# yweweler/single-speaker-tts

Hardware: AMD Instinct MI355X
Metric: mel-frames/sec (end-to-end text->waveform incl. 60-iter Griffin-Lim, 64-utt LJ-Speech-shaped batch per GPU) (higher is better)
Workload: dtype f32

## Files before the change

### include/sstts_hip.h

```cpp
#ifndef SSTTS_HIP_H
#define SSTTS_HIP_H

#include <stddef.h>
#include <stdint.h>

#ifdef __cplusplus
extern "C" {
#endif

typedef struct tts_handle_s* tts_handle_t;

enum tts_status {
    TTS_OK = 0,
    TTS_ERR_INVALID = -1,
    TTS_ERR_NOT_LOADED = -2,
    TTS_ERR_HIP = -3,
    TTS_ERR_DB_RANGE = -4,
    TTS_ERR_UNSUPPORTED = -5
};

typedef struct tts_config {
    int32_t struct_size;
    int32_t vocabulary_size;
    int32_t embedding_size;
// ... 129 lines not shown

int tts_synthesize_host(tts_handle_t h, const int32_t* ids_host, int B, int Ts, const tts_synth_params_t* p,
                        int* ticket);
int tts_wait_host(tts_handle_t h, int ticket, const float** wav_host, size_t* n_floats);
int tts_wait_host_outputs(tts_handle_t h, int ticket, const float** linear_host, size_t* n_linear, const float** align_host,
                          size_t* n_align);

int tts_profile_reset(tts_handle_t h);
int tts_decoder_kernel_choice(tts_handle_t h, int B, int T_sent, int pipelined);
int tts_debug_workspace(tts_handle_t h, const char* name, void** dptr, size_t* bytes);
int tts_debug_gl_plan(int T, int B, int win_length, int hop_length, int n_workers, int* items, int max_items, int* ring_frames);
int tts_debug_gl_plan_ragged(const int32_t* n_frames, int B, int win_length, int hop_length, int n_workers,
                             int* items, int max_items, int* ring_frames);
int tts_debug_gemm(tts_handle_t h, const float* A, const float* Wt, float* C, int M, int N, int Cin, int ktaps, int T,
                   int pool);
int tts_debug_hold(tts_handle_t h, int n_wgs, int lds_kb, double ms);
int tts_profile_get(tts_handle_t h, const char* stage, float* ms_total, int64_t* launches);
int tts_device_info(tts_handle_t h, char uuid_hex[33], int* n_compute_units);

#ifdef __cplusplus
}
#endif
#endif
```

### single-speaker-tts_amd/_hip.py

```python
import ctypes
import os
from ctypes import (POINTER, byref, c_char_p, c_float, c_int, c_int32, c_int64, c_size_t, c_uint64,
                    c_void_p)

import numpy as np

_HERE = os.path.dirname(os.path.abspath(__file__))
LIB_PATH = os.environ.get('SSTTS_HIP_LIB') or os.path.join(_HERE, 'libsstts_hip.so')

TTS_OK = 0
TTS_ERR_INVALID = -1
TTS_ERR_NOT_LOADED = -2
TTS_ERR_HIP = -3
TTS_ERR_DB_RANGE = -4
TTS_ERR_UNSUPPORTED = -5


class TtsError(RuntimeError):
    def __init__(self, code, msg):
        super().__init__('sstts_hip error {}: {}'.format(code, msg))
        self.code = code


class TtsConfig(ctypes.Structure):
# ... 74 lines not shown
    'tts_default_feature_params': (c_int, [POINTER(TtsFeatureParams)]),
    'tts_plan_features': (c_int, [c_void_p, c_void_p, c_void_p, c_int, POINTER(TtsFeatureParams), c_void_p]),
    'tts_extract_features': (c_int, [c_void_p, c_void_p, c_void_p, c_int, POINTER(TtsFeatureParams), c_void_p, c_void_p,
                                     c_void_p]),
    'tts_synthesize': (c_int, [c_void_p, c_void_p, c_int, c_int, POINTER(TtsSynthParams), c_void_p, c_void_p,
                               c_void_p, c_void_p, c_void_p]),
    'tts_synthesize_host': (c_int, [c_void_p, c_void_p, c_int, c_int, POINTER(TtsSynthParams), POINTER(c_int)]),
    'tts_wait_host': (c_int, [c_void_p, c_int, POINTER(c_void_p), POINTER(c_size_t)]),
    'tts_wait_host_outputs': (c_int, [c_void_p, c_int, POINTER(c_void_p), POINTER(c_size_t), POINTER(c_void_p), POINTER(c_size_t)]),
    'tts_profile_reset': (c_int, [c_void_p]),
    'tts_profile_get': (c_int, [c_void_p, c_char_p, POINTER(c_float), POINTER(c_int64)]),
    'tts_decoder_kernel_choice': (c_int, [c_void_p, c_int, c_int, c_int]),
    'tts_debug_workspace': (c_int, [c_void_p, c_char_p, POINTER(c_void_p), POINTER(c_size_t)]),
    'tts_debug_hold': (c_int, [c_void_p, c_int, c_int, ctypes.c_double]),
    'tts_debug_gemm': (c_int, [c_void_p, c_void_p, c_void_p, c_void_p, c_int, c_int, c_int, c_int, c_int, c_int]),
    'tts_debug_gl_plan': (c_int, [c_int, c_int, c_int, c_int, c_int, POINTER(c_int), c_int, POINTER(c_int)]),
    'tts_debug_gl_plan_ragged': (c_int, [POINTER(c_int32), c_int, c_int, c_int, c_int, POINTER(c_int), c_int, POINTER(c_int)]),
    'tts_device_info': (c_int, [c_void_p, c_char_p, POINTER(c_int)]),
}

_lib = None


def exported_symbols():
    return sorted(_PROTOTYPES)


def load_library(path=None):
    global _lib
    if _lib is not None and path is None:
# ... 551 lines not shown
```

### single-speaker-tts_amd/csrc/api_handle.hip

```cpp
#include "api_internal.h"

namespace tts_api {
thread_local std::string g_create_error;
const char* const kStageNames[ST_COUNT] = {"encoder", "decoder", "postnet", "denorm", "gl_iter", "gl_final", "debug_gemm", "eval_loss", "features"};
}

namespace tts_api {


int fail(tts_handle_t h, int code, const std::string& msg) {
    if (h) h->err = msg;
    else g_create_error = msg;
    return code;
}


const char* kAtt = "decoder2/decoder/output_projection_wrapper/multi_rnn_cell/cell_0/attention_wrapper";

const char* kMrc = "decoder2/decoder/output_projection_wrapper/multi_rnn_cell";


std::string bn_name(int i) {
    return i == 0 ? std::string("batch_normalization") : "batch_normalization_" + std::to_string(i);
}
// ... 635 lines not shown
int tts_set_option(tts_handle_t h, const char* key, int value) {
    DeviceScope dev_scope(h);
    if (!h || !key) return TTS_ERR_INVALID;
    if (!std::strcmp(key, "use_graph")) {
        int have = 0;
        if (value && !(value == 2 && h->debug_hooks) && !graph_runtime_ok(&have))
            return fail(h, TTS_ERR_UNSUPPORTED,
                        "use_graph: this process runs the library on HIP runtime " + std::to_string(have) + ", older than the " +
                        std::to_string(HIP_VERSION) + " it was built with (a libamdhip64 loaded before the library, e.g. the one "
                        "PyTorch bundles); hipGraph replays of the decoder are wrong there (csrc/api_internal.h, `use_graph`) -- the "
                        "launches are enqueued directly instead");
        h->use_graph = value;
    }
    else if (!std::strcmp(key, "profile")) h->profile = value;
    else if (!std::strcmp(key, "fused_tail")) h->fused_tail = value;
    else if (!std::strcmp(key, "persistent_decoder")) {
        if (value != h->persistent_decoder) {
            int rc = sync_all(h);
            if (rc) return rc;
        }
        h->persistent_decoder = value;
    }
    else if (!std::strcmp(key, "gl_pair")) h->gl_pair = value;
    else if (!std::strcmp(key, "gl_momentum")) {
        if (value < 0 || value > 999) return fail(h, TTS_ERR_INVALID, "gl_momentum: thousandths of the momentum, 0 .. 999");
        h->gl_momentum = value;
    }
    else if (!std::strcmp(key, "gl_wide_from")) h->gl_wide = value < -2 ? -2 : value;
    else if (!std::strcmp(key, "pd_ws")) {
        if (value != h->pd_ws) {
// ... 350 lines not shown
```

### single-speaker-tts_amd/csrc/api_internal.h

```cpp
#pragma once
#include <cmath>
#include <cstdio>
#include <cstring>
#include <memory>
#include <mutex>
#include <optional>
#include <string>
#include <utility>
#include <vector>
#include "decoder.h"
#include "griffin_lim.h"
#include "tts_common.h"
#include <algorithm>
#include <map>

namespace tts_api {
using namespace tts;


constexpr int TTS_MAX_N_MELS = 1024;
constexpr int TTS_MAX_FIELD = 1 << 20;
constexpr long long TTS_MAX_WEIGHT_FLOATS = (1ll << 30) - 5;

extern thread_local std::string g_create_error;
// ... 156 lines not shown
    }
};

}
using namespace tts_api;

struct tts_handle_s {
    tts_config_t cfg;
    int device = 0;
    hipStream_t stream = nullptr;
    bool own_stream = false;
    std::string err;
    int use_graph = 0;
    int fused_tail = 1;
    bool tail_configured = false;
    int profile = 0;
    int pipeline = 1;
    int reserve_cus = 32;
    int hold_lds_kb = 64;
    int enc_stream = 1;
    CallPipeline pl;
    int persistent_decoder = 1;
    int pd_ws = 1;
    bool ws_configured = false;
    int gl_pair = 3;
    int gl_momentum = 0;
    int gl_wide = -1;
    int n_cus_dev = 0;
    bool pd_configured = false;
    int debug_hooks = 0;
// ... 199 lines not shown
```

### single-speaker-tts_amd/csrc/api_pipeline.hip

```cpp
#include "api_internal.h"

namespace tts_api {


int gl_wide_from(tts_handle_t h, int B, int Ts, int n_steps, int T, int n_iter) {
    if (h->gl_wide == -2 || h->reserve_cus <= 0) return -1;
    const int pd = pd_choice(h, B, Ts, h->reserve_cus, true);
    if (pd == 0) return -1;
    if (h->gl_wide >= 0) return h->gl_wide;
    if (pd != 2) return -1;
    const int per_launch = h->gl_momentum > 0 ? 1 : (h->gl_pair < 1 ? 1 : (h->gl_pair > 3 ? 3 : h->gl_pair));
    if (h->n_cus_dev != 256 || h->n_cus_dev - h->reserve_cus < 16) return -1;
    const double launch_ms = 3.125e-6 * (double)B * T * per_launch * 224.0 / (double)(h->n_cus_dev - h->reserve_cus);
    const double step_ms = (0.0356 + 0.0089 * (double)Ts / 150.0) * (h->cfg.force_cudnn ? 0.038 / 0.045 : 1.0);
    const double dec_ms = step_ms * n_steps + 0.1;
    const int n_launches = (n_iter + per_launch - 1) / per_launch;
    const int from = (int)std::ceil((dec_ms + 0.5 * launch_ms + 0.1) / launch_ms);
    return from <= n_launches ? from : -1;
}

struct SynthCall {
    const int32_t* ids;
    int B, Ts;
    const tts_synth_params_t* sp;
// ... 171 lines not shown
    args.project_later = k.pipelined;
    args.parity = parity;
    args.keys = k.pipelined ? k.keys_ahead : nullptr;
    if ((rc = decoder_impl(h, k.memory, B, Ts, k.sp->n_steps, k.mel, k.align_out, nullptr, args, &k.proj))) return rc;
    if (k.pipelined) HIPCHK(h, pl.dec_done[parity].record(pl.front));
    else if (pl.front) HIPCHK(h, pl.serial_done.record(on.main_stream));
    return TTS_OK;
}

static int synth_main(tts_handle_t h, SynthCall& k) {
    auto& pl = h->pl;
    const tts_synth_params_t* sp = k.sp;
    const int B = k.B, T = k.T, parity = k.parity;
    int rc = TTS_OK;
    const bool phase_on_front = k.gl_streaming && k.pipelined && sp->n_iter >= 0 && (k.init_phase != nullptr || sp->n_iter == 0);
    if (k.pipelined) {
        if (k.hold_flag) HIPCHK(h, hipMemsetAsync(k.hold_flag, 1, sizeof(int), pl.front));
        if (phase_on_front) {
            HIPCHK(h, pl.gl_done[parity].wait(pl.front));
            HIPCHK(h, launch_phase_init(pl.front, k.init_phase, sp->seed, k.phase_pair[0], B, k.F, T, k.FP));
        }
        HIPCHK(h, pl.front_done.record(pl.front));
        HIPCHK(h, pl.front_done.wait(h->stream));
    }
    if (k.proj && (rc = run_single(h, *k.proj))) return rc;
    if (pl.encs) HIPCHK(h, pl.gap[parity].record(h->stream));
    int* db_flag = nullptr;
    if (denorm_can_assert(sp->ref_db, sp->max_db) && (rc = denorm_flag_arm(h, &db_flag))) return rc;
    if ((rc = postnet_impl(h, k.mel, B, T, k.linear_out, k.magi, sp->ref_db, sp->max_db, sp->power, db_flag))) return rc;
    if (db_flag && (rc = denorm_flag_read(h))) return rc;
    if (pl.front) HIPCHK(h, pl.post_done[parity].record(h->stream));
    const int wide_from = (k.pipelined && k.gl_streaming) ? gl_wide_from(h, B, k.Ts, sp->n_steps, T, sp->n_iter) : -1;
    pl.gl_wide_used[parity] = wide_from >= 0;
    if (k.gl_streaming)
        rc = gl_run(h, k.magi, k.init_phase, sp->seed, B, T, sp->n_iter, sp->win_length, sp->hop_length, h->cfg.n_fft, k.wav, nullptr,
                    sp->peak_normalize != 0, k.pipelined, k.phase_pair, phase_on_front, wide_from);
    else
        rc = gl_run_generic(h, k.magi, k.init_phase, sp->seed, B, T, sp->n_iter, sp->win_length, sp->hop_length, h->cfg.n_fft, k.wav,
                            nullptr, sp->peak_normalize != 0);
    if (pl.front && !rc) HIPCHK(h, pl.gl_done[parity].record(h->stream));
    return rc;
}

static int synthesize_impl(tts_handle_t h, const int32_t* ids, int B, int Ts, const tts_synth_params_t* sp, const float* init_phase,
                           float* wav, float* mel_out, float* align_out, float* linear_out, const StageArgs& host) {
    int rc = check_ready(h);
    if (rc) return rc;
// ... 146 lines not shown
```

### single-speaker-tts_amd/csrc/api_stages.hip

```cpp
#include "api_internal.h"

namespace tts_api {


int run_cbhg(tts_handle_t h, const CbhgWeights& w, const char* tag, const float* x, int B, int T, float* out,
             int64_t* launches) {
    const tts_config_t& c = h->cfg;
    const int M = B * T;
    const int NB = w.n_banks, NF = w.n_filters;
    const int U = c.n_highway_units, H = c.n_gru_units;
    const std::string t(tag);
    WS(h, (t + ".bank").c_str(), float, (size_t)M * NB * NF, bank);
    WS(h, (t + ".p1").c_str(), float, (size_t)M * w.proj_filters[0], p1);
    WS(h, (t + ".p2").c_str(), float, (size_t)M * w.proj_filters[1], p2);
    WS(h, (t + ".hw0").c_str(), float, (size_t)M * U, hw0);
    WS(h, (t + ".hw1").c_str(), float, (size_t)M * U, hw1);
    WS(h, (t + ".xproj").c_str(), float, (size_t)M * 6 * H, xproj);

    for (int k0 = 0; k0 < NB; k0 += TTS_GEMM_MAX_GROUPS) {
        GemmBatch b;
        std::memset(&b, 0, sizeof(b));
        const int ng = std::min(TTS_GEMM_MAX_GROUPS, NB - k0);
        for (int i = 0; i < ng; ++i) {
            const int k = k0 + ng - 1 - i;
            b.g[i] = conv_group(x, w.c_in, k + 1, T, w.bank_wt[k], w.bank_b[k], w.bank_scale[k], w.bank_shift[k], bank,
                                NB * NF, k * NF, M, NF, ACT_RELU, 0);
        }
        HIPCHK(h, launch_gemm(h->stream, b, ng));
        ++*launches;
    }
    {
        GemmGroup g = conv_group(bank, NB * NF, 3, T, w.proj_wt[0], w.proj_b[0], w.proj_scale[0], w.proj_shift[0], p1,
                                 w.proj_filters[0], 0, M, w.proj_filters[0], ACT_RELU, 1);
        const int slices = gemm_splitk_slices(g.K);
        if (slices > 1) {
            WS(h, (t + ".splitk").c_str(), float, (size_t)slices * M * g.N, part);
            HIPCHK(h, launch_gemm_splitk(h->stream, g, slices, part));
            ++*launches;
        } else {
            int rc = run_single(h, g);
            if (rc) return rc;
        }
        ++*launches;
    }
    {
        GemmGroup g = conv_group(p1, w.proj_filters[0], 3, T, w.proj_wt[1], w.proj_b[1], w.proj_scale[1],
                                 w.proj_shift[1], p2, w.proj_filters[1], 0, M, w.proj_filters[1], ACT_NONE, 0);
        g.R = x;
// ... 798 lines not shown
        return fail(h, TTS_ERR_DB_RANGE,
                    "\"conversion.decibel_to_magnitude\" was asked to convert a dB value smaller -100 dB.");
    return TTS_OK;
}

}

extern "C" {

int tts_encoder_forward(tts_handle_t h, const int32_t* ids, int B, int Ts, float* memory) {
    DeviceScope dev_scope(h);
    int rc = check_ready(h);
    if (rc) return rc;
    if (!ids || !memory || B < 1 || Ts < 1) return fail(h, TTS_ERR_INVALID, "encoder_forward: bad arguments");
    if ((rc = standalone_begin(h))) return rc;
    if ((rc = encoder_impl(h, ids, B, Ts, memory))) return rc;
    return standalone_end(h);
}

int tts_decoder_forward(tts_handle_t h, const float* memory, int B, int Ts, int n_steps, float* mel,
                        float* alignments) {
    DeviceScope dev_scope(h);
    int rc = check_ready(h);
    if (rc) return rc;
    if (!memory || !mel || B < 1 || Ts < 1 || n_steps < 1) return fail(h, TTS_ERR_INVALID, "decoder_forward: bad arguments");
    if ((rc = standalone_begin(h))) return rc;
    if ((rc = decoder_impl(h, memory, B, Ts, n_steps, mel, alignments))) return rc;
    return standalone_end(h);
}


// ... 4 lines not shown
    if (rc) return rc;
    if (!memory || !mel_target || !mel || B < 1 || Ts < 1 || n_steps < 1)
        return fail(h, TTS_ERR_INVALID, "decoder_forward_teacher: bad arguments");
    if ((uintptr_t)mel_target & 15) return fail(h, TTS_ERR_INVALID, "decoder_forward_teacher: mel_target must be 16-byte aligned");
    if ((long long)n_steps * h->cfg.reduction > (1 << 24) || (long long)n_steps * h->cfg.reduction * h->cfg.n_mels > 0x7FFFFFFFll)
        return fail(h, TTS_ERR_INVALID, "decoder_forward_teacher: sizes out of range");
    if ((rc = standalone_begin(h))) return rc;
    if ((rc = decoder_impl(h, memory, B, Ts, n_steps, mel, alignments, mel_target))) return rc;
    return standalone_end(h);
}


int tts_postnet_forward(tts_handle_t h, const float* mel, int B, int T, float* linear) {
    DeviceScope dev_scope(h);
    if (!linear) return fail(h, TTS_ERR_INVALID, "postnet_forward: bad arguments");
    return postnet_impl(h, mel, B, T, linear, nullptr, 0.f, 0.f, 1.f);
}


int tts_evaluate(tts_handle_t h, const int32_t* ids, int B, int Ts, int n_steps, const float* mel_target,
                 const float* linear_target, float* losses, double* l1_sums, float* mel, float* alignments, float* linear) {
    DeviceScope dev_scope(h);
    int rc = check_ready(h);
    if (rc) return rc;
    if (!ids || !mel_target || !linear_target || !losses || B < 1 || Ts < 1 || n_steps < 1)
        return fail(h, TTS_ERR_INVALID, "evaluate: bad arguments (ids, both targets and losses are required; B, Ts, n_steps >= 1)");
    const tts_config_t& c = h->cfg;
    const int T = n_steps * c.reduction, F = 1 + c.n_fft / 2;
    if ((long long)n_steps * c.reduction > (1 << 24) || (double)B * T * F >= 9.0e18)
        return fail(h, TTS_ERR_INVALID, "evaluate: sizes out of range");
    for (const void* p : {(const void*)mel_target, (const void*)linear_target, (const void*)mel, (const void*)linear,
// ... 285 lines not shown
    std::vector<int4> v;
    int slots = 0;
    const int n = gl_plan_items_ragged(n_frames, T_max, B, win_length, hop_length, n_workers, n_stage, 0, 0, &v, &slots);
    if (ring_frames) *ring_frames = ring;
    for (int k = 0; k < n && k < max_items; ++k) {
        items[4 * k] = v[k].x; items[4 * k + 1] = v[k].y; items[4 * k + 2] = v[k].z; items[4 * k + 3] = v[k].w;
    }
    return n;
}


int tts_debug_gemm(tts_handle_t h, const float* A, const float* Wt, float* C, int M, int N, int Cin, int ktaps, int T,
                   int pool) {
    DeviceScope dev_scope(h);
    if (!h || !A || !Wt || !C || M < 1 || N < 1 || Cin < 4 || (Cin & 3) || ktaps < 1 || T < 1 || M % T) return TTS_ERR_INVALID;
    GemmGroup g = conv_group(A, Cin, ktaps, T, Wt, nullptr, nullptr, nullptr, C, N, 0, M, N, ACT_NONE, pool);
    ProfScope ps(h, ST_DEBUG_GEMM, 1);
    const int slices = gemm_splitk_slices(g.K);
    if (slices > 1) {
        WS(h, "debug.splitk", float, (size_t)slices * M * N, part);
        HIPCHK(h, launch_gemm_splitk(h->stream, g, slices, part));
        return TTS_OK;
    }
    return run_single(h, g);
}


int tts_debug_hold(tts_handle_t h, int n_wgs, int lds_kb, double ms) {
    DeviceScope dev_scope(h);
    if (!h || n_wgs < 1 || lds_kb < 1 || lds_kb > 160) return TTS_ERR_INVALID;
    if (!h->debug_hooks) return fail(h, TTS_ERR_INVALID, "tts_debug_hold: a diagnostic; set the option \"debug_hooks\" to 1 on this handle first");
    static hipStream_t dbg = nullptr;
    static int* never = nullptr;
    static std::mutex dbg_mutex;
    std::lock_guard<std::mutex> lock(dbg_mutex);
    if (!dbg) {
        HIPCHK(h, hipStreamCreateWithFlags(&dbg, hipStreamNonBlocking));
        HIPCHK(h, hipMalloc(reinterpret_cast<void**>(&never), sizeof(int)));
        HIPCHK(h, hipMemset(never, 0, sizeof(int)));
// ... 8 lines not shown
```

### single-speaker-tts_amd/csrc/gemm_f32.hip

```cpp
#include "tts_common.h"
#include <cstring>
#include <type_traits>

namespace tts {

#define GEMM_NUM_VGPR 80
#define GEMM_NUM_VGPR_POOL 128
#define BM 128
#define BN 128
#define BK 32
#define LDS_LD (BK + 4)
typedef __bf16 bf16x8_t __attribute__((ext_vector_type(8)));
__device__ __forceinline__ void split3(float x, unsigned& h, unsigned& m, unsigned& l) {
    h = __float_as_uint(x);
    const float r1 = x - __uint_as_float(h & 0xFFFF0000u);
    m = __float_as_uint(r1);
    const float r2 = r1 - __uint_as_float(m & 0xFFFF0000u);
    l = __float_as_uint(r2);
}
__device__ __forceinline__ unsigned pack_hi(unsigned a, unsigned b) { return __builtin_amdgcn_perm(b, a, 0x07060302u); }
__device__ __forceinline__ void store_split4(unsigned char* img, int row, int kq, float4 v) {
    unsigned h[4], m[4], l[4];
    split3(v.x, h[0], m[0], l[0]);
    split3(v.y, h[1], m[1], l[1]);
    split3(v.z, h[2], m[2], l[2]);
    split3(v.w, h[3], m[3], l[3]);
    const int off = (row * 4 + ((kq >> 1) ^ ((row >> 2) & 3))) * 16 + (kq & 1) * 8;
    *reinterpret_cast<uint2*>(img + off) = make_uint2(pack_hi(h[0], h[1]), pack_hi(h[2], h[3]));
    *reinterpret_cast<uint2*>(img + BM * 64 + off) = make_uint2(pack_hi(m[0], m[1]), pack_hi(m[2], m[3]));
    *reinterpret_cast<uint2*>(img + 2 * BM * 64 + off) = make_uint2(pack_hi(l[0], l[1]), pack_hi(l[2], l[3]));
}

__device__ __forceinline__ float4 max4(float4 a, float4 b) {
    return make_float4(fmaxf(a.x, b.x), fmaxf(a.y, b.y), fmaxf(a.z, b.z), fmaxf(a.w, b.w));
}

template <bool DENORM, bool POOL>
__device__ __forceinline__ void gemm_body(const GemmBatch& batch) {
    const GemmGroup& g = batch.g[blockIdx.z];
    const int M = g.M, N = g.N, K = g.K;
    const int nyb = gridDim.y;
    const int lin = blockIdx.x + gridDim.x * blockIdx.y;
    const int xcd = lin & 7, seq = lin >> 3;
    const int m_blk = (seq / nyb) * 8 + xcd;
    const int m0 = m_blk * BM;
    const int n0 = (seq % nyb) * BN;
    if (n0 >= N || m0 >= M) return;

    __shared__ __attribute__((aligned(16))) unsigned char As_lds[3 * BM * 64];
    __shared__ __attribute__((aligned(16))) unsigned char Bs_lds[3 * BN * 64];
    unsigned char* const As = As_lds;
    unsigned char* const Bs = Bs_lds;

    const int tid = threadIdx.x;
    const int lane = tid & 63;
    const int wave = tid >> 6;
    const int wm = wave >> 1, wn = wave & 1;
    const int li = lane & 31, lh = lane >> 5;

    typedef __attribute__((__vector_size__(4 * sizeof(unsigned)))) unsigned u32x4_t;
    const __amdgpu_buffer_rsrc_t a_rs = __builtin_amdgcn_make_buffer_rsrc(const_cast<float*>(g.A), 0, (int)0xFFFFFFF0u, 0x00020000);
    const __amdgpu_buffer_rsrc_t b_rs = __builtin_amdgcn_make_buffer_rsrc(const_cast<float*>(g.Wt), 0, (int)0xFFFFFFF0u, 0x00020000);
    auto buf4 = [](const __amdgpu_buffer_rsrc_t& rs, unsigned byte_off) {
        return __builtin_bit_cast(float4, __builtin_amdgcn_raw_buffer_load_b128(rs, (int)byte_off, 0, 0));
    };
    int a_off[4];
    int a_t[4];
    bool a_ok[4];
    int b_off[4];
    bool b_ok[4];
    const int kq = tid & 7;
#pragma unroll
    for (int i = 0; i < 4; ++i) {
        const int row = (tid >> 3) + 32 * i;
        const int m = m0 + (POOL ? 4 * (tid >> 3) + i : row);
        a_ok[i] = m < M;
        const int mm = a_ok[i] ? m : 0;
        a_t[i] = mm % g.T;
        if (g.gather) {
            const int id = g.gather[mm];
            const bool in_table = (unsigned)id < (unsigned)g.gather_rows;
            a_ok[i] = a_ok[i] && in_table;
            a_off[i] = (in_table ? id : 0) * g.lda;
        } else {
            a_off[i] = (mm - g.padl) * g.lda;
        }
        const int n = n0 + row;
        b_ok[i] = n < N;
        b_off[i] = (b_ok[i] ? n : 0) * K;
    }

    float4 ra[4], rb[4];
    float4 ra4 = make_float4(0.f, 0.f, 0.f, 0.f);
    unsigned pool_own = 0, pool_nxt = 0;
    bool pool_raw = false;
    const int ktaps = K / g.Cin;
    const bool tap_inner = ktaps > 1 && (g.Cin % BK) == 0;
    const bool uniform_tap = ktaps == 1 || tap_inner;
    int cur_tap = 0, cur_kb = 0;
    int my_tap = 0, my_ch = 0;
    {
        const int k_first = g.kt1 > 0 ? g.kt0 : 0;
        if (tap_inner) {
// ... 44 lines not shown
                    const float4 v = buf4(a_rs, (mine || succ) ? (unsigned)(base + kk) * 4u : 0xFFFFFFFFu);
                    if (j < 4) ra[j] = v;
                    else ra4 = v;
                }
                pool_own = (own[0] ? 1u : 0u) | (own[1] ? 2u : 0u) | (own[2] ? 4u : 0u) | (own[3] ? 8u : 0u);
                pool_nxt = (nxt[0] ? 1u : 0u) | (nxt[1] ? 2u : 0u) | (nxt[2] ? 4u : 0u) | (nxt[3] ? 8u : 0u);
#pragma unroll
                for (int i = 0; i < 4; ++i)
                    rb[i] = buf4(b_rs, (b_ok[i] && kin) ? (unsigned)(b_off[i] + kk) * 4u : 0xFFFFFFFFu);
            } else {
#pragma unroll
                for (int i = 0; i < 4; ++i) {
                    const bool ok = kin && ((tapmask[i] >> tap) & 1u);
                    const unsigned off = ok ? (unsigned)(a_off[i] + kk) * 4u : 0xFFFFFFFFu;
                    ra[i] = buf4(a_rs, off);
                    rb[i] = buf4(b_rs, (b_ok[i] && kin) ? (unsigned)(b_off[i] + kk) * 4u : 0xFFFFFFFFu);
                }
            }
            if (tap_inner) {
                if (++cur_tap == ktaps) { cur_tap = 0; cur_kb += BK - (ktaps - 1) * g.Cin; }
                else cur_kb += g.Cin;
            } else if (uniform_tap) {
                cur_kb += BK;
            } else if (!POOL) {
                my_ch += BK;
                while (my_ch >= g.Cin) { my_ch -= g.Cin; ++my_tap; }
            }
            return;
        }
        const int kk = kt + 4 * kq;
        const bool kin = kk < K;
        const int tap = kk / g.Cin;
#pragma unroll
        for (int i = 0; i < 4; ++i) {
            const int ts = a_t[i] - g.padl + tap;
            const bool ok = a_ok[i] && kin && ts >= 0 && ts < g.T;
            const unsigned off = ok ? (unsigned)(a_off[i] + kk) * 4u : 0xFFFFFFFFu;
            float4 v = buf4(a_rs, off);
            if (POOL) v = max4(v, buf4(a_rs, (ok && ts + 1 < g.T) ? off + (unsigned)g.lda * 4u : off));
            ra[i] = v;
            rb[i] = buf4(b_rs, (b_ok[i] && kin) ? (unsigned)(b_off[i] + kk) * 4u : 0xFFFFFFFFu);
        }
    };
    auto store_tile = [&]() {
        if (POOL && pool_raw) {
            const float4 z = make_float4(0.f, 0.f, 0.f, 0.f);
#pragma unroll
            for (int i = 0; i < 4; ++i) {
                const float4 x = ((pool_own >> i) & 1u) ? ra[i] : z;
                const float4 nx = i < 3 ? ra[i < 3 ? i + 1 : 3] : ra4;
                ra[i] = ((pool_nxt >> i) & 1u) ? max4(x, nx) : x;
            }
        }
#pragma unroll
        for (int i = 0; i < 4; ++i) {
            const int row = (tid >> 3) + 32 * i;
            const int arow = POOL ? 4 * (tid >> 3) + i : row;
            store_split4(As, arow, kq, ra[i]);
            store_split4(Bs, row, kq, rb[i]);
        }
    };

    bool blk_live[2][2];
#pragma unroll
    for (int tm = 0; tm < 2; ++tm)
#pragma unroll
        for (int tn = 0; tn < 2; ++tn)
            blk_live[tm][tn] = (m0 + wm * 64 + tm * 32 < M) && (n0 + wn * 64 + tn * 32 < N);
    f32x16 acc[2][2];
#pragma unroll
    for (int i = 0; i < 2; ++i)
#pragma unroll
        for (int j = 0; j < 2; ++j)
#pragma unroll
            for (int r = 0; r < 16; ++r) acc[i][j][r] = 0.f;

    const int k_begin = g.kt1 > 0 ? g.kt0 : 0;
    const int k_end = g.kt1 > 0 ? g.kt1 : K;
    auto mma_tile = [&](auto edge_c) {
        constexpr bool EDGE = decltype(edge_c)::value;
#pragma unroll
        for (int q = 0; q < 2; ++q) {
            const int ch = 2 * q + lh;
            uint4 fa[2][3];
#pragma unroll
            for (int tm = 0; tm < 2; ++tm) {
                const int row = wm * 64 + tm * 32 + li;
                const int off = (row * 4 + (ch ^ ((row >> 2) & 3))) * 16;
#pragma unroll
                for (int sp = 0; sp < 3; ++sp) fa[tm][sp] = *reinterpret_cast<const uint4*>(As + sp * BM * 64 + off);
            }
#pragma unroll
            for (int tn = 0; tn < 2; ++tn) {
                const int row = wn * 64 + tn * 32 + li;
                const int off = (row * 4 + (ch ^ ((row >> 2) & 3))) * 16;
                uint4 fb[3];
#pragma unroll
                for (int sp = 0; sp < 3; ++sp) fb[sp] = *reinterpret_cast<const uint4*>(Bs + sp * BN * 64 + off);
#pragma unroll
                for (int tm = 0; tm < 2; ++tm) {
                    if (EDGE && !blk_live[tm][tn]) continue;
#define GEMM_MMA(SA, SB)                                                                                              \
                    acc[tm][tn] = __builtin_amdgcn_mfma_f32_32x32x16_bf16(__builtin_bit_cast(bf16x8_t, fa[tm][SA]),    \
                                                                          __builtin_bit_cast(bf16x8_t, fb[SB]), acc[tm][tn], 0, 0, 0);
                    GEMM_MMA(0, 2) GEMM_MMA(2, 0) GEMM_MMA(1, 1) GEMM_MMA(0, 1) GEMM_MMA(1, 0) GEMM_MMA(0, 0)
#undef GEMM_MMA
                }
            }
        }
    };
    auto k_loop = [&](auto edge_c) {
        load_tile(k_begin);
        for (int kt = k_begin; kt < k_end; kt += BK) {
            store_tile();
            __syncthreads();
            if (kt + BK < k_end) load_tile(kt + BK);
            mma_tile(edge_c);
            __syncthreads();
        }
    };
    if (blk_live[0][0] && blk_live[0][1] && blk_live[1][0] && blk_live[1][1]) k_loop(std::false_type{});
    else k_loop(std::true_type{});

    if (g.epi == EPI_HIGHWAY) {
        const int span = (n0 + wn * 64) >> 6;
        const int unit = span * 32 + li;
        const int nh = n0 + wn * 64 + li;
        const float bh = g.bias ? g.bias[nh] : 0.f;
        const float bt = g.bias ? g.bias[nh + 32] : 0.f;
#pragma unroll
        for (int tm = 0; tm < 2; ++tm)
#pragma unroll
            for (int r = 0; r < 16; ++r) {
                const int m = m0 + wm * 64 + tm * 32 + (r & 3) + 8 * (r >> 2) + 4 * lh;
                if (m < M) {
                    const float hh = fmaxf(acc[tm][0][r] + bh, 0.f);
                    const float tt = sigmoidf_(acc[tm][1][r] + bt);
                    const float x = g.A[(size_t)m * g.lda + unit];
                    g.C[(size_t)m * g.ldc + g.coff + unit] = hh * tt + x * (1.0f - tt);
                }
            }
        return;
    }
#pragma unroll
    for (int tn = 0; tn < 2; ++tn) {
        const int n = n0 + wn * 64 + tn * 32 + li;
        if (n >= N) {
            if (DENORM && g.C2 && n < g.N2) {
#pragma unroll
                for (int tm = 0; tm < 2; ++tm)
#pragma unroll
                    for (int r = 0; r < 16; ++r) {
                        const int m = m0 + wm * 64 + tm * 32 + (r & 3) + 8 * (r >> 2) + 4 * lh;
                        if (m < M) g.C2[(size_t)m * g.ldc2 + n] = 0.f;
                    }
            }
            continue;
        }
        const float bv = g.bias ? g.bias[n] : 0.f;
        const float sc = g.scale ? g.scale[n] : 1.f;
        const float sh = g.scale ? g.shift[n] : 0.f;
#pragma unroll
        for (int tm = 0; tm < 2; ++tm)
#pragma unroll
            for (int r = 0; r < 16; ++r) {
                const int m = m0 + wm * 64 + tm * 32 + (r & 3) + 8 * (r >> 2) + 4 * lh;
                if (m < M) {
                    float v = apply_act(acc[tm][tn][r] + bv, g.act);
                    v = v * sc + sh;
                    if (g.R) v += g.R[(size_t)m * g.ldr + n];
                    if (!DENORM || g.C) g.C[(size_t)m * g.ldc + g.coff + n] = v;
                    if (DENORM && g.C2) {
                        const float db = denorm_db(v, g.d_ref, g.d_range);
                        if (g.d_flag && db < -100.0f) *g.d_flag = 1;
                        g.C2[(size_t)m * g.ldc2 + n] = db_pow(db, g.d_pow);
                    }
                }
            }
    }
}

template <bool DENORM>
__global__ __launch_bounds__(256) __attribute__((amdgpu_num_vgpr(GEMM_NUM_VGPR))) void gemm_f32_kernel(GemmBatch batch) {
    gemm_body<DENORM, false>(batch);
}
__global__ __launch_bounds__(256) __attribute__((amdgpu_num_vgpr(GEMM_NUM_VGPR_POOL))) void gemm_f32_pool_kernel(GemmBatch batch) {
    gemm_body<false, true>(batch);
}

hipError_t launch_gemm(hipStream_t s, const GemmBatch& b, int n_groups) {
    int max_n = 0;
    for (int i = 0; i < n_groups; ++i) {
        const GemmGroup& g = b.g[i];
        max_n = g.N > max_n ? g.N : max_n;
        const size_t a_rows = g.gather ? (size_t)g.gather_rows : (size_t)g.M + (size_t)(g.pool ? 1 : 0);
        if (a_rows * (size_t)g.lda * 4 >= 0xFFFFFFF0ull || (size_t)g.N * (size_t)g.K * 4 >= 0xFFFFFFF0ull) return hipErrorInvalidValue;
    }
    const int m_blocks = (b.g[0].M + BM - 1) / BM;
    dim3 grid((m_blocks + 7) / 8 * 8, (max_n + BN - 1) / BN, n_groups);
    bool denorm = false;
    for (int i = 0; i < n_groups; ++i) denorm = denorm || b.g[i].C2 != nullptr;
    bool pool = false;
    for (int i = 0; i < n_groups; ++i) pool = pool || b.g[i].pool != 0;
    for (int i = 0; i < n_groups; ++i)
        if (pool && (!b.g[i].pool || b.g[i].C2)) return hipErrorInvalidValue;
    if (pool) hipLaunchKernelGGL(gemm_f32_pool_kernel, grid, dim3(256), 0, s, b);
    else if (denorm) hipLaunchKernelGGL((gemm_f32_kernel<true>), grid, dim3(256), 0, s, b);
    else hipLaunchKernelGGL((gemm_f32_kernel<false>), grid, dim3(256), 0, s, b);
    return hipGetLastError();
}

__global__ void splitk_reduce_kernel(const float* __restrict__ partial, int slices, GemmGroup g) {
    const size_t i = (size_t)blockIdx.x * blockDim.x + threadIdx.x;
    const size_t total = (size_t)g.M * g.N;
    if (i >= total) return;
    const int m = (int)(i / g.N), n = (int)(i % g.N);
    float v = 0.f;
    for (int s = 0; s < slices; ++s) v += partial[(size_t)s * total + i];
    v = apply_act(v + (g.bias ? g.bias[n] : 0.f), g.act);
    if (g.scale) v = v * g.scale[n] + g.shift[n];
    if (g.R) v += g.R[(size_t)m * g.ldr + n];
    g.C[(size_t)m * g.ldc + g.coff + n] = v;
// ... 28 lines not shown
```

### single-speaker-tts_amd/csrc/tts_common.h

```cpp
#pragma once
#include <hip/hip_runtime.h>
#include <stdint.h>
#include <stddef.h>
#include <map>
#include <string>
#include <vector>

#include "../../include/sstts_hip.h"

namespace tts {

typedef float f32x4 __attribute__((ext_vector_type(4)));
typedef float f32x16 __attribute__((ext_vector_type(16)));

enum Act { ACT_NONE = 0, ACT_RELU = 1, ACT_SIGMOID = 2, ACT_TANH = 3 };
enum Epi { EPI_STD = 0, EPI_HIGHWAY = 1 };

__device__ __forceinline__ float sigmoidf_(float x) { return __builtin_amdgcn_rcpf(1.0f + __expf(-x)); }
__device__ __forceinline__ double wave_sum_f64(double v) {
#pragma unroll
    for (int o = 32; o > 0; o >>= 1) v += __shfl_xor(v, o);
    return v;
}
__device__ __forceinline__ void split_f64(double v, float* hi, float* lo) {
// ... 39 lines not shown
    const float* bias;
    const float* scale;
    const float* shift;
    const float* R;
    float* C;
    int M, N, K;
    int lda, T, Cin, padl, pool;
    int ldc, coff, ldr;
    int act, epi;
    float* C2;
    int ldc2, N2;
    float d_ref, d_range, d_pow;
    int* d_flag;
    int kt0, kt1;
};
#define TTS_GEMM_MAX_GROUPS 16
struct GemmBatch {
    GemmGroup g[TTS_GEMM_MAX_GROUPS];
};
hipError_t launch_gemm(hipStream_t s, const GemmBatch& b, int n_groups);
hipError_t launch_gemm_splitk(hipStream_t s, const GemmGroup& g, int slices, float* partial);
int gemm_splitk_slices(int K);

hipError_t launch_bigru(hipStream_t s, const float* xproj, int xld, const float* wrec, float* out,
                        int B, int T, int H, int cudnn);
size_t bigru_wrec_floats(int H, int cudnn);

#define CBHG_TAIL_MAX_HW 8
struct CbhgTailParams {
    const float* X; int ldx; int c_in;
    const float* lifter_wt; const float* lifter_b;
    const float* hw_wt[CBHG_TAIL_MAX_HW]; const float* hw_b[CBHG_TAIL_MAX_HW]; int n_hw;
    const float* gru_wt; const float* gru_b;
    float* hw_out;
    float* xproj;
// ... 20 lines not shown
```

Before: 4.417 million.

## Fuse CBHG max-pool into bank GEMM epilogue, add narrow GEMM tile, hoist projection

```diff
diff --git a/include/sstts_hip.h b/include/sstts_hip.h
--- a/include/sstts_hip.h
+++ b/include/sstts_hip.h
@@ -167,6 +167,8 @@
                              int* items, int max_items, int* ring_frames);
 int tts_debug_gemm(tts_handle_t h, const float* A, const float* Wt, float* C, int M, int N, int Cin, int ktaps, int T,
                    int pool);
+int tts_debug_gemm_ex(tts_handle_t h, const float* A, const float* Wt, float* C, int M, int N, int Cin, int ktaps, int T,
+                      int pool, const float* bias, const float* scale, const float* shift, const float* R, int act, int wide);
 int tts_debug_hold(tts_handle_t h, int n_wgs, int lds_kb, double ms);
 int tts_profile_get(tts_handle_t h, const char* stage, float* ms_total, int64_t* launches);
 int tts_device_info(tts_handle_t h, char uuid_hex[33], int* n_compute_units);
diff --git a/single-speaker-tts_amd/_hip.py b/single-speaker-tts_amd/_hip.py
--- a/single-speaker-tts_amd/_hip.py
+++ b/single-speaker-tts_amd/_hip.py
@@ -112,6 +112,8 @@
     'tts_debug_workspace': (c_int, [c_void_p, c_char_p, POINTER(c_void_p), POINTER(c_size_t)]),
     'tts_debug_hold': (c_int, [c_void_p, c_int, c_int, ctypes.c_double]),
     'tts_debug_gemm': (c_int, [c_void_p, c_void_p, c_void_p, c_void_p, c_int, c_int, c_int, c_int, c_int, c_int]),
+    'tts_debug_gemm_ex': (c_int, [c_void_p, c_void_p, c_void_p, c_void_p, c_int, c_int, c_int, c_int, c_int, c_int,
+                                  c_void_p, c_void_p, c_void_p, c_void_p, c_int, c_int]),
     'tts_debug_gl_plan': (c_int, [c_int, c_int, c_int, c_int, c_int, POINTER(c_int), c_int, POINTER(c_int)]),
     'tts_debug_gl_plan_ragged': (c_int, [POINTER(c_int32), c_int, c_int, c_int, c_int, POINTER(c_int), c_int, POINTER(c_int)]),
     'tts_device_info': (c_int, [c_void_p, c_char_p, POINTER(c_int)]),
diff --git a/single-speaker-tts_amd/csrc/api_handle.hip b/single-speaker-tts_amd/csrc/api_handle.hip
--- a/single-speaker-tts_amd/csrc/api_handle.hip
+++ b/single-speaker-tts_amd/csrc/api_handle.hip
@@ -673,6 +673,8 @@
     }
     else if (!std::strcmp(key, "profile")) h->profile = value;
     else if (!std::strcmp(key, "fused_tail")) h->fused_tail = value;
+    else if (!std::strcmp(key, "pool_in_loader")) h->pool_in_loader = value ? 1 : 0;
+    else if (!std::strcmp(key, "keep_bank")) h->keep_bank_opt = value ? 1 : 0;
     else if (!std::strcmp(key, "persistent_decoder")) {
         if (value != h->persistent_decoder) {
             int rc = sync_all(h);
diff --git a/single-speaker-tts_amd/csrc/api_internal.h b/single-speaker-tts_amd/csrc/api_internal.h
--- a/single-speaker-tts_amd/csrc/api_internal.h
+++ b/single-speaker-tts_amd/csrc/api_internal.h
@@ -194,6 +194,9 @@
     int use_graph = 0;
     int fused_tail = 1;
     bool tail_configured = false;
+    int pool_in_loader = 0;
+    bool keep_bank = false;
+    int keep_bank_opt = 1;
     int profile = 0;
     int pipeline = 1;
     int reserve_cus = 32;
diff --git a/single-speaker-tts_amd/csrc/api_pipeline.hip b/single-speaker-tts_amd/csrc/api_pipeline.hip
--- a/single-speaker-tts_amd/csrc/api_pipeline.hip
+++ b/single-speaker-tts_amd/csrc/api_pipeline.hip
@@ -209,7 +209,14 @@
     const int B = k.B, T = k.T, parity = k.parity;
     int rc = TTS_OK;
     const bool phase_on_front = k.gl_streaming && k.pipelined && sp->n_iter >= 0 && (k.init_phase != nullptr || sp->n_iter == 0);
+    const int wide_from = (k.pipelined && k.gl_streaming) ? gl_wide_from(h, B, k.Ts, sp->n_steps, T, sp->n_iter) : -1;
     if (k.pipelined) {
+        if (k.proj && wide_from >= 0) {
+            StreamScope on(h);
+            on.aim(pl.front);
+            if ((rc = run_single(h, *k.proj))) return rc;
+            k.proj.reset();
+        }
         if (k.hold_flag) HIPCHK(h, hipMemsetAsync(k.hold_flag, 1, sizeof(int), pl.front));
         if (phase_on_front) {
             HIPCHK(h, pl.gl_done[parity].wait(pl.front));
@@ -225,7 +232,6 @@
     if ((rc = postnet_impl(h, k.mel, B, T, k.linear_out, k.magi, sp->ref_db, sp->max_db, sp->power, db_flag))) return rc;
     if (db_flag && (rc = denorm_flag_read(h))) return rc;
     if (pl.front) HIPCHK(h, pl.post_done[parity].record(h->stream));
-    const int wide_from = (k.pipelined && k.gl_streaming) ? gl_wide_from(h, B, k.Ts, sp->n_steps, T, sp->n_iter) : -1;
     pl.gl_wide_used[parity] = wide_from >= 0;
     if (k.gl_streaming)
         rc = gl_run(h, k.magi, k.init_phase, sp->seed, B, T, sp->n_iter, sp->win_length, sp->hop_length, h->cfg.n_fft, k.wav, nullptr,
diff --git a/single-speaker-tts_amd/csrc/api_stages.hip b/single-speaker-tts_amd/csrc/api_stages.hip
--- a/single-speaker-tts_amd/csrc/api_stages.hip
+++ b/single-speaker-tts_amd/csrc/api_stages.hip
@@ -10,7 +10,17 @@
     const int NB = w.n_banks, NF = w.n_filters;
     const int U = c.n_highway_units, H = c.n_gru_units;
     const std::string t(tag);
-    WS(h, (t + ".bank").c_str(), float, (size_t)M * NB * NF, bank);
+    const bool pool_store = !h->pool_in_loader;
+    float* bank = nullptr;
+    float* bankp = nullptr;
+    if (!pool_store || h->keep_bank) {
+        WS(h, (t + ".bank").c_str(), float, (size_t)M * NB * NF, bank_ws);
+        bank = bank_ws;
+    }
+    if (pool_store) {
+        WS(h, (t + ".bankp").c_str(), float, (size_t)M * NB * NF, bankp_ws);
+        bankp = bankp_ws;
+    }
     WS(h, (t + ".p1").c_str(), float, (size_t)M * w.proj_filters[0], p1);
     WS(h, (t + ".p2").c_str(), float, (size_t)M * w.proj_filters[1], p2);
     WS(h, (t + ".hw0").c_str(), float, (size_t)M * U, hw0);
@@ -23,15 +33,18 @@
         const int ng = std::min(TTS_GEMM_MAX_GROUPS, NB - k0);
         for (int i = 0; i < ng; ++i) {
             const int k = k0 + ng - 1 - i;
-            b.g[i] = conv_group(x, w.c_in, k + 1, T, w.bank_wt[k], w.bank_b[k], w.bank_scale[k], w.bank_shift[k], bank,
-                                NB * NF, k * NF, M, NF, ACT_RELU, 0);
+            b.g[i] = conv_group(x, w.c_in, k + 1, T, w.bank_wt[k], w.bank_b[k], w.bank_scale[k], w.bank_shift[k],
+                                pool_store ? bankp : bank, NB * NF, k * NF, M, NF, ACT_RELU,
+                                pool_store ? GEMM_POOL_STORE : GEMM_POOL_NONE);
+            if (pool_store && bank) { b.g[i].C2 = bank; b.g[i].ldc2 = NB * NF; }
         }
         HIPCHK(h, launch_gemm(h->stream, b, ng));
         ++*launches;
     }
     {
-        GemmGroup g = conv_group(bank, NB * NF, 3, T, w.proj_wt[0], w.proj_b[0], w.proj_scale[0], w.proj_shift[0], p1,
-                                 w.proj_filters[0], 0, M, w.proj_filters[0], ACT_RELU, 1);
+        GemmGroup g = conv_group(pool_store ? bankp : bank, NB * NF, 3, T, w.proj_wt[0], w.proj_b[0], w.proj_scale[0],
+                                 w.proj_shift[0], p1, w.proj_filters[0], 0, M, w.proj_filters[0], ACT_RELU,
+                                 pool_store ? GEMM_POOL_NONE : GEMM_POOL_LOADER);
         const int slices = gemm_splitk_slices(g.K);
         if (slices > 1) {
             WS(h, (t + ".splitk").c_str(), float, (size_t)slices * M * g.N, part);
@@ -860,7 +873,10 @@
     if (rc) return rc;
     if (!ids || !memory || B < 1 || Ts < 1) return fail(h, TTS_ERR_INVALID, "encoder_forward: bad arguments");
     if ((rc = standalone_begin(h))) return rc;
-    if ((rc = encoder_impl(h, ids, B, Ts, memory))) return rc;
+    h->keep_bank = h->keep_bank_opt != 0;
+    rc = encoder_impl(h, ids, B, Ts, memory);
+    h->keep_bank = false;
+    if (rc) return rc;
     return standalone_end(h);
 }
 
@@ -895,7 +911,10 @@
 int tts_postnet_forward(tts_handle_t h, const float* mel, int B, int T, float* linear) {
     DeviceScope dev_scope(h);
     if (!linear) return fail(h, TTS_ERR_INVALID, "postnet_forward: bad arguments");
-    return postnet_impl(h, mel, B, T, linear, nullptr, 0.f, 0.f, 1.f);
+    h->keep_bank = h->keep_bank_opt != 0;
+    const int rc = postnet_impl(h, mel, B, T, linear, nullptr, 0.f, 0.f, 1.f);
+    h->keep_bank = false;
+    return rc;
 }
 
 
@@ -1211,6 +1230,7 @@
                    int pool) {
     DeviceScope dev_scope(h);
     if (!h || !A || !Wt || !C || M < 1 || N < 1 || Cin < 4 || (Cin & 3) || ktaps < 1 || T < 1 || M % T) return TTS_ERR_INVALID;
+    if (pool != GEMM_POOL_NONE && pool != GEMM_POOL_LOADER) return TTS_ERR_INVALID;
     GemmGroup g = conv_group(A, Cin, ktaps, T, Wt, nullptr, nullptr, nullptr, C, N, 0, M, N, ACT_NONE, pool);
     ProfScope ps(h, ST_DEBUG_GEMM, 1);
     const int slices = gemm_splitk_slices(g.K);
@@ -1220,6 +1240,26 @@
         return TTS_OK;
     }
     return run_single(h, g);
+}
+
+
+int tts_debug_gemm_ex(tts_handle_t h, const float* A, const float* Wt, float* C, int M, int N, int Cin, int ktaps, int T,
+                      int pool, const float* bias, const float* scale, const float* shift, const float* R, int act, int wide) {
+    DeviceScope dev_scope(h);
+    if (!h || !A || !Wt || !C || M < 1 || N < 1 || Cin < 4 || (Cin & 3) || ktaps < 1 || T < 1 || M % T || pool < 0 || pool > 2 ||
+        (scale == nullptr) != (shift == nullptr) || (pool && R))
+        return TTS_ERR_INVALID;
+    if (!h->debug_hooks) return fail(h, TTS_ERR_INVALID, "tts_debug_gemm_ex: a diagnostic; set the option \"debug_hooks\" to 1 on this handle first");
+    GemmGroup g = conv_group(A, Cin, ktaps, T, Wt, bias, scale, shift, C, N, 0, M, N, act ? ACT_RELU : ACT_NONE, pool);
+    g.R = R;
+    g.ldr = N;
+    if (gemm_splitk_slices(g.K) > 1) return fail(h, TTS_ERR_UNSUPPORTED, "tts_debug_gemm_ex: a split-K shape (tts_debug_gemm runs those)");
+    ProfScope ps(h, ST_DEBUG_GEMM, 1);
+    GemmBatch b;
+    std::memset(&b, 0, sizeof(b));
+    b.g[0] = g;
+    HIPCHK(h, launch_gemm(h->stream, b, 1, wide != 0));
+    return TTS_OK;
 }
 
 
diff --git a/single-speaker-tts_amd/csrc/gemm_f32.hip b/single-speaker-tts_amd/csrc/gemm_f32.hip
--- a/single-speaker-tts_amd/csrc/gemm_f32.hip
+++ b/single-speaker-tts_amd/csrc/gemm_f32.hip
@@ -8,6 +8,7 @@
 #define GEMM_NUM_VGPR_POOL 128
 #define BM 128
 #define BN 128
+#define BN_NARROW 96
 #define BK 32
 #define LDS_LD (BK + 4)
 typedef __bf16 bf16x8_t __attribute__((ext_vector_type(8)));
@@ -19,7 +20,7 @@
     l = __float_as_uint(r2);
 }
 __device__ __forceinline__ unsigned pack_hi(unsigned a, unsigned b) { return __builtin_amdgcn_perm(b, a, 0x07060302u); }
-__device__ __forceinline__ void store_split4(unsigned char* img, int row, int kq, float4 v) {
+__device__ __forceinline__ void store_split4(unsigned char* img, int plane, int row, int kq, float4 v) {
     unsigned h[4], m[4], l[4];
     split3(v.x, h[0], m[0], l[0]);
     split3(v.y, h[1], m[1], l[1]);
@@ -27,35 +28,41 @@
     split3(v.w, h[3], m[3], l[3]);
     const int off = (row * 4 + ((kq >> 1) ^ ((row >> 2) & 3))) * 16 + (kq & 1) * 8;
     *reinterpret_cast<uint2*>(img + off) = make_uint2(pack_hi(h[0], h[1]), pack_hi(h[2], h[3]));
-    *reinterpret_cast<uint2*>(img + BM * 64 + off) = make_uint2(pack_hi(m[0], m[1]), pack_hi(m[2], m[3]));
-    *reinterpret_cast<uint2*>(img + 2 * BM * 64 + off) = make_uint2(pack_hi(l[0], l[1]), pack_hi(l[2], l[3]));
+    *reinterpret_cast<uint2*>(img + plane + off) = make_uint2(pack_hi(m[0], m[1]), pack_hi(m[2], m[3]));
+    *reinterpret_cast<uint2*>(img + 2 * plane + off) = make_uint2(pack_hi(l[0], l[1]), pack_hi(l[2], l[3]));
 }
 
 __device__ __forceinline__ float4 max4(float4 a, float4 b) {
     return make_float4(fmaxf(a.x, b.x), fmaxf(a.y, b.y), fmaxf(a.z, b.z), fmaxf(a.w, b.w));
 }
 
-template <bool DENORM, bool POOL>
+template <bool DENORM, bool POOL, bool PSTORE, bool NARROW>
 __device__ __forceinline__ void gemm_body(const GemmBatch& batch) {
+    static_assert(!(PSTORE && (DENORM || POOL || NARROW)) && !(NARROW && (DENORM || POOL)), "instantiations that exist");
+    constexpr int TBN = NARROW ? BN_NARROW : BN;
+    constexpr int WGN = NARROW ? 1 : 2, WGM = 4 / WGN;
+    constexpr int TMB = BM / WGM / 32, TNB = TBN / WGN / 32;
+    constexpr int B_LD = TBN / 32;
+    constexpr int M_STEP = PSTORE ? BM - 1 : BM;
     const GemmGroup& g = batch.g[blockIdx.z];
     const int M = g.M, N = g.N, K = g.K;
     const int nyb = gridDim.y;
     const int lin = blockIdx.x + gridDim.x * blockIdx.y;
     const int xcd = lin & 7, seq = lin >> 3;
     const int m_blk = (seq / nyb) * 8 + xcd;
-    const int m0 = m_blk * BM;
-    const int n0 = (seq % nyb) * BN;
+    const int m0 = m_blk * M_STEP;
+    const int n0 = (seq % nyb) * TBN;
     if (n0 >= N || m0 >= M) return;
 
     __shared__ __attribute__((aligned(16))) unsigned char As_lds[3 * BM * 64];
-    __shared__ __attribute__((aligned(16))) unsigned char Bs_lds[3 * BN * 64];
+    __shared__ __attribute__((aligned(16))) unsigned char Bs_lds[3 * TBN * 64];
     unsigned char* const As = As_lds;
     unsigned char* const Bs = Bs_lds;
 
     const int tid = threadIdx.x;
     const int lane = tid & 63;
     const int wave = tid >> 6;
-    const int wm = wave >> 1, wn = wave & 1;
+    const int wm = NARROW ? wave : wave >> 1, wn = NARROW ? 0 : wave & 1;
     const int li = lane & 31, lh = lane >> 5;
 
     typedef __attribute__((__vector_size__(4 * sizeof(unsigned)))) unsigned u32x4_t;
@@ -86,7 +93,7 @@
             a_off[i] = (mm - g.padl) * g.lda;
         }
         const int n = n0 + row;
-        b_ok[i] = n < N;
+        b_ok[i] = i < B_LD && n < N;
         b_off[i] = (b_ok[i] ? n : 0) * K;
     }
 
@@ -161,7 +168,7 @@
                     const bool ok = kin && ((tapmask[i] >> tap) & 1u);
                     const unsigned off = ok ? (unsigned)(a_off[i] + kk) * 4u : 0xFFFFFFFFu;
                     ra[i] = buf4(a_rs, off);
-                    rb[i] = buf4(b_rs, (b_ok[i] && kin) ? (unsigned)(b_off[i] + kk) * 4u : 0xFFFFFFFFu);
+                    if (i < B_LD) rb[i] = buf4(b_rs, (b_ok[i] && kin) ? (unsigned)(b_off[i] + kk) * 4u : 0xFFFFFFFFu);
                 }
             }
             if (tap_inner) {
@@ -186,7 +193,7 @@
             float4 v = buf4(a_rs, off);
             if (POOL) v = max4(v, buf4(a_rs, (ok && ts + 1 < g.T) ? off + (unsigned)g.lda * 4u : off));
             ra[i] = v;
-            rb[i] = buf4(b_rs, (b_ok[i] && kin) ? (unsigned)(b_off[i] + kk) * 4u : 0xFFFFFFFFu);
+            if (i < B_LD) rb[i] = buf4(b_rs, (b_ok[i] && kin) ? (unsigned)(b_off[i] + kk) * 4u : 0xFFFFFFFFu);
         }
     };
     auto store_tile = [&]() {
@@ -203,22 +210,26 @@
         for (int i = 0; i < 4; ++i) {
             const int row = (tid >> 3) + 32 * i;
             const int arow = POOL ? 4 * (tid >> 3) + i : row;
-            store_split4(As, arow, kq, ra[i]);
-            store_split4(Bs, row, kq, rb[i]);
+            store_split4(As, BM * 64, arow, kq, ra[i]);
+            if (i < B_LD) store_split4(Bs, TBN * 64, row, kq, rb[i]);
         }
     };
 
-    bool blk_live[2][2];
-#pragma unroll
-    for (int tm = 0; tm < 2; ++tm)
-#pragma unroll
-        for (int tn = 0; tn < 2; ++tn)
-            blk_live[tm][tn] = (m0 + wm * 64 + tm * 32 < M) && (n0 + wn * 64 + tn * 32 < N);
-    f32x16 acc[2][2];
-#pragma unroll
-    for (int i = 0; i < 2; ++i)
-#pragma unroll
-        for (int j = 0; j < 2; ++j)
+    const int wrow = wm * (TMB * 32), wcol = wn * (TNB * 32);
+    bool blk_live[TMB][TNB];
+    bool all_live = true;
+#pragma unroll
+    for (int tm = 0; tm < TMB; ++tm)
+#pragma unroll
+        for (int tn = 0; tn < TNB; ++tn) {
+            blk_live[tm][tn] = (m0 + wrow + tm * 32 < M) && (n0 + wcol + tn * 32 < N);
+            all_live = all_live && blk_live[tm][tn];
+        }
+    f32x16 acc[TMB][TNB];
+#pragma unroll
+    for (int i = 0; i < TMB; ++i)
+#pragma unroll
+        for (int j = 0; j < TNB; ++j)
 #pragma unroll
             for (int r = 0; r < 16; ++r) acc[i][j][r] = 0.f;
 
@@ -229,23 +240,23 @@
 #pragma unroll
         for (int q = 0; q < 2; ++q) {
             const int ch = 2 * q + lh;
-            uint4 fa[2][3];
-#pragma unroll
-            for (int tm = 0; tm < 2; ++tm) {
-                const int row = wm * 64 + tm * 32 + li;
+            uint4 fa[TMB][3];
+#pragma unroll
+            for (int tm = 0; tm < TMB; ++tm) {
+                const int row = wrow + tm * 32 + li;
                 const int off = (row * 4 + (ch ^ ((row >> 2) & 3))) * 16;
 #pragma unroll
                 for (int sp = 0; sp < 3; ++sp) fa[tm][sp] = *reinterpret_cast<const uint4*>(As + sp * BM * 64 + off);
             }
 #pragma unroll
-            for (int tn = 0; tn < 2; ++tn) {
-                const int row = wn * 64 + tn * 32 + li;
+            for (int tn = 0; tn < TNB; ++tn) {
+                const int row = wcol + tn * 32 + li;
                 const int off = (row * 4 + (ch ^ ((row >> 2) & 3))) * 16;
                 uint4 fb[3];
 #pragma unroll
-                for (int sp = 0; sp < 3; ++sp) fb[sp] = *reinterpret_cast<const uint4*>(Bs + sp * BN * 64 + off);
-#pragma unroll
-                for (int tm = 0; tm < 2; ++tm) {
+                for (int sp = 0; sp < 3; ++sp) fb[sp] = *reinterpret_cast<const uint4*>(Bs + sp * TBN * 64 + off);
+#pragma unroll
+                for (int tm = 0; tm < TMB; ++tm) {
                     if (EDGE && !blk_live[tm][tn]) continue;
 #define GEMM_MMA(SA, SB)                                                                                              \
                     acc[tm][tn] = __builtin_amdgcn_mfma_f32_32x32x16_bf16(__builtin_bit_cast(bf16x8_t, fa[tm][SA]),    \
@@ -266,9 +277,10 @@
             __syncthreads();
         }
     };
-    if (blk_live[0][0] && blk_live[0][1] && blk_live[1][0] && blk_live[1][1]) k_loop(std::false_type{});
+    if (all_live) k_loop(std::false_type{});
     else k_loop(std::true_type{});
 
+    if constexpr (!NARROW && !PSTORE) {
     if (g.epi == EPI_HIGHWAY) {
         const int span = (n0 + wn * 64) >> 6;
         const int unit = span * 32 + li;
@@ -289,16 +301,86 @@
             }
         return;
     }
-#pragma unroll
-    for (int tn = 0; tn < 2; ++tn) {
-        const int n = n0 + wn * 64 + tn * 32 + li;
+    }
+    if constexpr (PSTORE) {
+        int gz = blockIdx.z;
+        asm volatile("" : "+s"(gz));
+        const GemmGroup& ge = batch.g[gz];
+#pragma unroll
+        for (int tn = 0; tn < 2; ++tn) {
+            const int n = n0 + wn * 64 + tn * 32 + li;
+            const bool nok = n < N;
+            const float bv = (nok && ge.bias) ? ge.bias[n] : 0.f;
+            const float sc = (nok && ge.scale) ? ge.scale[n] : 1.f;
+            const float sh = (nok && ge.scale) ? ge.shift[n] : 0.f;
+#pragma unroll
+            for (int tm = 0; tm < 2; ++tm)
+#pragma unroll
+                for (int r = 0; r < 16; ++r) {
+                    float v = apply_act(acc[tm][tn][r] + bv, ge.act);
+                    v = v * sc + sh;
+                    acc[tm][tn][r] = v;
+                }
+        }
+        float* const xrow = reinterpret_cast<float*>(As);
+        if (wm == 1 && lh == 0) {
+#pragma unroll
+            for (int tn = 0; tn < 2; ++tn) xrow[(wn * 2 + tn) * 32 + li] = acc[0][tn][0];
+        }
+        __syncthreads();
+        unsigned last_bits[2];
+#pragma unroll
+        for (int tm = 0; tm < 2; ++tm) {
+            const int base = m0 + wm * 64 + tm * 32 + 4 * lh;
+            unsigned bits = 0;
+            if (ge.T >= 32) {
+                const int rem = ge.T - 1 - base % ge.T;
+#pragma unroll
+                for (int r = 0; r < 16; ++r) bits |= ((r & 3) + 8 * (r >> 2) == rem ? 1u : 0u) << r;
+            } else {
+#pragma unroll
+                for (int r = 0; r < 16; ++r) bits |= ((base + (r & 3) + 8 * (r >> 2) + 1) % ge.T == 0 ? 1u : 0u) << r;
+            }
+            last_bits[tm] = bits;
+        }
+#pragma unroll
+        for (int tn = 0; tn < 2; ++tn) {
+            const int n = n0 + wn * 64 + tn * 32 + li;
+            const bool nok = n < N;
+#pragma unroll
+            for (int tm = 0; tm < 2; ++tm) {
+                const float below = tm == 0 ? acc[1][tn][0] : (wm == 0 ? xrow[(wn * 2 + tn) * 32 + li] : 0.f);
+                float recv[4];
+#pragma unroll
+                for (int j = 0; j < 4; ++j) {
+                    const float send = lh ? acc[tm][tn][4 * j] : (j < 3 ? acc[tm][tn][j < 3 ? 4 * j + 4 : 0] : below);
+                    recv[j] = __shfl_xor(send, 32);
+                }
+#pragma unroll
+                for (int r = 0; r < 16; ++r) {
+                    const int lrow = wm * 64 + tm * 32 + (r & 3) + 8 * (r >> 2) + 4 * lh;
+                    const int m = m0 + lrow;
+                    if (nok && lrow < BM - 1 && m < M) {
+                        const float v = acc[tm][tn][r];
+                        const float nx = (r & 3) < 3 ? acc[tm][tn][(r & 3) < 3 ? r + 1 : r] : recv[r >> 2];
+                        ge.C[(size_t)m * ge.ldc + ge.coff + n] = ((last_bits[tm] >> r) & 1u) ? v : fmaxf(v, nx);
+                        if (ge.C2) ge.C2[(size_t)m * ge.ldc2 + ge.coff + n] = v;
+                    }
+                }
+            }
+        }
+        return;
+    }
+#pragma unroll
+    for (int tn = 0; tn < TNB; ++tn) {
+        const int n = n0 + wcol + tn * 32 + li;
         if (n >= N) {
             if (DENORM && g.C2 && n < g.N2) {
 #pragma unroll
-                for (int tm = 0; tm < 2; ++tm)
+                for (int tm = 0; tm < TMB; ++tm)
 #pragma unroll
                     for (int r = 0; r < 16; ++r) {
-                        const int m = m0 + wm * 64 + tm * 32 + (r & 3) + 8 * (r >> 2) + 4 * lh;
+                        const int m = m0 + wrow + tm * 32 + (r & 3) + 8 * (r >> 2) + 4 * lh;
                         if (m < M) g.C2[(size_t)m * g.ldc2 + n] = 0.f;
                     }
             }
@@ -308,10 +390,10 @@
         const float sc = g.scale ? g.scale[n] : 1.f;
         const float sh = g.scale ? g.shift[n] : 0.f;
 #pragma unroll
-        for (int tm = 0; tm < 2; ++tm)
+        for (int tm = 0; tm < TMB; ++tm)
 #pragma unroll
             for (int r = 0; r < 16; ++r) {
-                const int m = m0 + wm * 64 + tm * 32 + (r & 3) + 8 * (r >> 2) + 4 * lh;
+                const int m = m0 + wrow + tm * 32 + (r & 3) + 8 * (r >> 2) + 4 * lh;
                 if (m < M) {
                     float v = apply_act(acc[tm][tn][r] + bv, g.act);
                     v = v * sc + sh;
@@ -329,30 +411,43 @@
 
 template <bool DENORM>
 __global__ __launch_bounds__(256) __attribute__((amdgpu_num_vgpr(GEMM_NUM_VGPR))) void gemm_f32_kernel(GemmBatch batch) {
-    gemm_body<DENORM, false>(batch);
+    gemm_body<DENORM, false, false, false>(batch);
 }
 __global__ __launch_bounds__(256) __attribute__((amdgpu_num_vgpr(GEMM_NUM_VGPR_POOL))) void gemm_f32_pool_kernel(GemmBatch batch) {
-    gemm_body<false, true>(batch);
-}
-
-hipError_t launch_gemm(hipStream_t s, const GemmBatch& b, int n_groups) {
+    gemm_body<false, true, false, false>(batch);
+}
+__global__ __launch_bounds__(256) __attribute__((amdgpu_num_vgpr(GEMM_NUM_VGPR))) void gemm_f32_poolstore_kernel(GemmBatch batch) {
+    gemm_body<false, false, true, false>(batch);
+}
+__global__ __launch_bounds__(256) __attribute__((amdgpu_num_vgpr(GEMM_NUM_VGPR))) void gemm_f32_narrow_kernel(GemmBatch batch) {
+    gemm_body<false, false, false, true>(batch);
+}
+
+hipError_t launch_gemm(hipStream_t s, const GemmBatch& b, int n_groups, bool force_wide) {
     int max_n = 0;
+    bool denorm = false, plain_epi = true;
+    const int pool = b.g[0].pool;
+    if (pool != GEMM_POOL_NONE && pool != GEMM_POOL_LOADER && pool != GEMM_POOL_STORE) return hipErrorInvalidValue;
     for (int i = 0; i < n_groups; ++i) {
         const GemmGroup& g = b.g[i];
         max_n = g.N > max_n ? g.N : max_n;
-        const size_t a_rows = g.gather ? (size_t)g.gather_rows : (size_t)g.M + (size_t)(g.pool ? 1 : 0);
+        const size_t a_rows = g.gather ? (size_t)g.gather_rows : (size_t)g.M + (size_t)(g.pool == GEMM_POOL_LOADER ? 1 : 0);
         if (a_rows * (size_t)g.lda * 4 >= 0xFFFFFFF0ull || (size_t)g.N * (size_t)g.K * 4 >= 0xFFFFFFF0ull) return hipErrorInvalidValue;
-    }
-    const int m_blocks = (b.g[0].M + BM - 1) / BM;
-    dim3 grid((m_blocks + 7) / 8 * 8, (max_n + BN - 1) / BN, n_groups);
-    bool denorm = false;
-    for (int i = 0; i < n_groups; ++i) denorm = denorm || b.g[i].C2 != nullptr;
-    bool pool = false;
-    for (int i = 0; i < n_groups; ++i) pool = pool || b.g[i].pool != 0;
-    for (int i = 0; i < n_groups; ++i)
-        if (pool && (!b.g[i].pool || b.g[i].C2)) return hipErrorInvalidValue;
-    if (pool) hipLaunchKernelGGL(gemm_f32_pool_kernel, grid, dim3(256), 0, s, b);
+        if (g.pool != pool) return hipErrorInvalidValue;
+        if (pool == GEMM_POOL_LOADER && g.C2) return hipErrorInvalidValue;
+        if (pool == GEMM_POOL_STORE && (g.epi != EPI_STD || g.R || g.kt1 > 0 || g.T < 1 || g.M % g.T)) return hipErrorInvalidValue;
+        denorm = denorm || (pool == GEMM_POOL_NONE && g.C2 != nullptr);
+        plain_epi = plain_epi && g.epi == EPI_STD;
+    }
+    const int m_step = pool == GEMM_POOL_STORE ? BM - 1 : BM;
+    const int m_blocks = (b.g[0].M + m_step - 1) / m_step;
+    const bool narrow = !force_wide && max_n <= BN_NARROW && pool == GEMM_POOL_NONE && !denorm && plain_epi;
+    const int bn = narrow ? BN_NARROW : BN;
+    dim3 grid((m_blocks + 7) / 8 * 8, (max_n + bn - 1) / bn, n_groups);
+    if (pool == GEMM_POOL_LOADER) hipLaunchKernelGGL(gemm_f32_pool_kernel, grid, dim3(256), 0, s, b);
+    else if (pool == GEMM_POOL_STORE) hipLaunchKernelGGL(gemm_f32_poolstore_kernel, grid, dim3(256), 0, s, b);
     else if (denorm) hipLaunchKernelGGL((gemm_f32_kernel<true>), grid, dim3(256), 0, s, b);
+    else if (narrow) hipLaunchKernelGGL(gemm_f32_narrow_kernel, grid, dim3(256), 0, s, b);
     else hipLaunchKernelGGL((gemm_f32_kernel<false>), grid, dim3(256), 0, s, b);
     return hipGetLastError();
 }
diff --git a/single-speaker-tts_amd/csrc/tts_common.h b/single-speaker-tts_amd/csrc/tts_common.h
--- a/single-speaker-tts_amd/csrc/tts_common.h
+++ b/single-speaker-tts_amd/csrc/tts_common.h
@@ -77,11 +77,14 @@
     int* d_flag;
     int kt0, kt1;
 };
+#define GEMM_POOL_NONE 0
+#define GEMM_POOL_LOADER 1
+#define GEMM_POOL_STORE 2
 #define TTS_GEMM_MAX_GROUPS 16
 struct GemmBatch {
     GemmGroup g[TTS_GEMM_MAX_GROUPS];
 };
-hipError_t launch_gemm(hipStream_t s, const GemmBatch& b, int n_groups);
+hipError_t launch_gemm(hipStream_t s, const GemmBatch& b, int n_groups, bool force_wide = false);
 hipError_t launch_gemm_splitk(hipStream_t s, const GemmGroup& g, int slices, float* partial);
 int gemm_splitk_slices(int K);
 
```

Result: no change. 4.453 million, median of 6 (+0.8%).
